# Vasilispapg/CVML-GoalNet

Hardware: AMD Instinct MI355X
Metric: training clips/sec at batch 64, 16-frame 224² clips; logit MAE vs CPU ref (higher is better)
Workload: dtype f32; 1 GPU; AVM train step (forward + broadcast-MSE + backward + fused Adam), 64 clips x 16 frames = 1024 frames of 3x224x224 + 30x30 MFCC per GPU; dropout live (device masks), BatchNorm train mode; frames_per_gpu=1024, h=224, w=224, parallelism=dp1, ddp_semantics=local BN + local MSE per rank, gradient mean (standard DDP), params=1286754369

## Files before the change

__graft_entry__.py:

```python
from __future__ import annotations

import glob
import os
import subprocess
import sys

ROOT = os.path.dirname(os.path.abspath(__file__))
PKG = os.path.join(ROOT, "cvml_goalnet_amd")
CSRC = os.path.join(PKG, "csrc")
LIB = os.path.join(PKG, "libgoalnet_hip.so")
HIPCC = os.environ.get("HIPCC", "/opt/rocm/bin/hipcc")
FLAGS = ["--offload-arch=gfx950", "-O3", "-std=c++17", "-fPIC", "-Wall", "-Wno-unused-function"]


def _stale(target, sources):
    if not os.path.exists(target):
        return True
    t = os.path.getmtime(target)
    return any(os.path.getmtime(s) > t for s in sources)


def build(force: bool = False) -> None:
    srcs = sorted(glob.glob(os.path.join(CSRC, "*.hip")))
    hdrs = sorted(glob.glob(os.path.join(CSRC, "*.h"))) + [os.path.join(ROOT, "include", h) for h in ("goalnet_hip.h", "goalnet_loss.h", "goalnet_epoch.h", "goalnet_optim.h", "goalnet_ema.h")]
    objdir = os.path.join(CSRC, "build")
    os.makedirs(objdir, exist_ok=True)
    objs = []
    procs = []
    for s in srcs:
        o = os.path.join(objdir, os.path.basename(s)[:-4] + ".o")
        objs.append(o)
        if force or _stale(o, [s] + hdrs):
            procs.append((s, subprocess.Popen([HIPCC, *FLAGS, "-c", s, "-o", o])))
    for s, p in procs:
        if p.wait() != 0:
            raise RuntimeError(f"hipcc failed on {s}")
    if force or procs or _stale(LIB, objs):
        subprocess.check_call([HIPCC, "--offload-arch=gfx950", "-shared", "-fPIC", "-o", LIB, *objs])
    if ROOT not in sys.path:
# ... 54 lines not shown
```

cvml_goalnet_amd/_lib.py:

```python
from __future__ import annotations

import ctypes
import os
from ctypes import c_char_p, c_double, c_float, c_int, c_int32, c_int64, c_size_t, c_uint32, c_uint64, c_void_p

_HERE = os.path.dirname(os.path.abspath(__file__))
LIB_PATH = os.environ.get("GOALNET_LIB_PATH") or os.path.join(_HERE, "libgoalnet_hip.so")
ABI_VERSION = 7
STAT_PARTS = 1024
ADAM_RANGES_MAX = 32

P = c_void_p


class RowCopy(ctypes.Structure):
    _fields_ = [("src", c_void_p), ("dst", c_void_p), ("row_bytes", c_int64), ("nrows", c_int), ("gather", c_int), ("cursor", c_void_p),
                ("cursor_bias", c_int64)]


class RowCopyIndexed(ctypes.Structure):
    _fields_ = [("src", c_void_p), ("dst", c_void_p), ("row_bytes", c_int64), ("nrows", c_int), ("gather", c_int), ("cursor", c_void_p),
                ("cursor_bias", c_int64), ("indexed", c_int), ("table_rows", c_int64)]


# ... 173 lines not shown

OPTIM_PROTOTYPES = {
    "goalnet_grad_sumsq_ws_bytes": (c_size_t, [ctypes.POINTER(OptimRange), c_int]),
    "goalnet_grad_sumsq": (c_int, [P, ctypes.POINTER(OptimRange), c_int, P, P, c_size_t, P]),
    "goalnet_optim_step_dev_ranges": (c_int, [P, P, P, P, ctypes.POINTER(OptimRange), c_int, ctypes.POINTER(OptimOpts), P, c_float, P,
                                              P, c_int64, c_int64, c_int, P, P]),
    "goalnet_optim_lr": (c_int, [ctypes.POINTER(OptimOpts), P, P, P]),
}
SCHEDULES = {"constant": 0, "cosine": 1, "step": 2}

EMA_PROTOTYPES = {
    "goalnet_ema_update_dev_ranges": (c_int, [P, P, ctypes.POINTER(AdamRange), c_int, ctypes.POINTER(EmaOpts), P, c_int64, P, P]),
    "goalnet_swap_ranges": (c_int, [P, P, ctypes.POINTER(AdamRange), c_int, P]),
}

_lib = None


class GoalnetError(RuntimeError):
    pass


def load():
    global _lib
    if _lib is not None:
        return _lib
    if not os.path.exists(LIB_PATH):
        raise GoalnetError(
            f"{LIB_PATH} not found: build it with `python -c 'import __graft_entry__ as g; g.build()'`. "
            "There is no CPU / eager fallback for the AVM hot path.")
    lib = ctypes.CDLL(LIB_PATH)
    for name, (res, args) in (*PROTOTYPES.items(), *LOSS_PROTOTYPES.items(), *EPOCH_PROTOTYPES.items(), *OPTIM_PROTOTYPES.items(),
                              *EMA_PROTOTYPES.items()):
        fn = getattr(lib, name)
        fn.restype = res
        fn.argtypes = args
    v = lib.goalnet_abi_version()
    if v != ABI_VERSION:
        raise GoalnetError(f"libgoalnet_hip.so ABI {v} != expected {ABI_VERSION}")
    _lib = lib
    return lib


def check(rc: int, what: str = ""):
    if rc != 0:
        msg = load().goalnet_last_error()
        raise GoalnetError(f"{what}: rc={rc}: {msg.decode() if msg else ''}")
```

cvml_goalnet_amd/avm.py:

```python
from __future__ import annotations

import contextlib
import math
import os
from typing import List, Optional

import torch
import torch.nn as nn
from torch.nn.parameter import UninitializedParameter

from . import ops
from ._lib import GoalnetError
from .synth import BASE_SEED, DROP_P, TID_DROP

F32 = torch.float32
BN_EPS = 1e-5
BN_MOMENTUM = 0.1
_ALIGN = 64


class _LazyFlags:

    def requires_grad_(self, requires_grad: bool = True):
        for p in self.parameters():
# ... 57 lines not shown
            torch.cuda.current_stream().wait_event(ev)

    def join(self):
        if self.enabled and self.forked:
            torch.cuda.current_stream().wait_stream(self.side)
            self.forked = False
        self.keep.clear()


class _Bwd:

    def __init__(self, model, train, fork):
        self.model, self.train, self.fork = model, train, fork
        self.scratch = {}
        self.dbias = {}
        self.T = train.__contains__

    def any_T(self, *layers):
        return any(f"{layer}.{leaf}" in self.train for layer in layers for leaf in ("weight", "bias"))

    def G(self, name):
        m = self.model
        if name in self.train:
            return m._gflat(name)
        s = m.spec(name)
        if s.kind in ("ohwi", "lin5") and name != "visbl.conv1.weight":
            raise GoalnetError(f"a backward that does not train {name} asked for its gradient")
        t = self.scratch.get(name)
        if t is None:
            t = self.scratch[name] = torch.empty(s.numel, dtype=F32, device=m._device)
# ... 32 lines not shown
    if env is None or env in ("", "1"):
        return frozenset("a")
    if env == "0":
        return frozenset()
    return frozenset(ch for ch in env.lower() if ch in "a")


def epi_fuse_dw_adam(n, *, plain, synced, precision, train_w5, shadowed, inspected, forced, pieces):
    if forced is False or "a" not in pieces:
        return False
    if inspected and forced is not True:
        return False
    if not (plain and not synced and precision == "fp32" and train_w5 and not shadowed):
        return False
    if n <= EPI_FUSE_SKINNY_ROWS:
        return False
    return forced is True or n >= EPI_FUSE_MIN_ROWS


def optim_step_path(optim, *, sharded):
    if optim is None or optim.trivial:
        return False
    if sharded:
        raise GoalnetError("optimizer options (weight decay, clipping, schedules) are not built for ddp.GradSync(shard_linear5=True): "
                           "a rank holds only its slice of linear5.weight's gradient; use a plain GradSync")
    return True


def ema_step_path(ema, *, sharded):
    if ema is None:
# ... 85 lines not shown
        self._materialized = False
        self.grad_sync = None
        self.stat_sync = None
        self.grad_bf16 = os.environ.get("GOALNET_DZ16", "1") != "0"
        self.act_bf16 = os.environ.get("GOALNET_P16", "1") != "0"
        env = os.environ.get
        self.x6_off = env("GOALNET_X6_OFF") == "1"
        self.x6_linear5 = env("GOALNET_X6_LINEAR5", "1") != "0"
        self.x3_wgrad2 = env("GOALNET_X3_WGRAD2", "1") != "0"
        self.x3_dgrad2 = env("GOALNET_X3_DGRAD2", "1") != "0"
        self.mlp_fused = env("GOALNET_MLP_FUSED", "1") != "0"
        self.small_bn = env("GOALNET_SMALL_BN", "1") != "0"
        self.force_bf5 = env("GOALNET_FORCE_BF5") == "1"
        self.overlap_pair = env("GOALNET_OVERLAP_PAIR", "1") != "0"
        self.epi_fuse = None
        self.epi_fused_dw = 0
        self.keep_ctx = False
        self.last_ctx = None
        self.last_used_w5b = False
        self._side_stream = None
        self.overlap_rows = int(os.environ.get("GOALNET_OVERLAP_ROWS", "64"))
        _ol = os.environ.get("GOALNET_OVERLAP_LARGE")
        self.overlap_large = _ol == "1"
        self.overlap_auto = _ol is None
        self.time_labels = None
        self.kernel_events = None

    @property
    def precision(self) -> str:
        return self._precision
# ... 543 lines not shown

    def _block_bwd(self, bwd, dbn, ctx, i, n, hc, wc, c):
        dev, G, bias = self._device, bwd.G, bwd.T(f"visbl.conv{i}.bias")
        p, idx, st = ctx[f"p{i}"], ctx[f"idx{i}"], ctx[f"st{i}"]
        npix = n * (hc - 2) * (wc - 2)
        small = self._small_bn(dbn, p, n, hc, wc, c) and not (self._half and i > 1)
        frozen = ctx["eval"]
        if small:
            coef3 = torch.empty(3 * c, dtype=F32, device=dev)
            (ops.bn_bwd_reduce_small_eval if frozen else ops.bn_bwd_reduce_small)(
                dbn, p, st[0], st[1], self._pflat(f"visbl.bnorm{i}.weight"), G(f"visbl.bnorm{i}.weight"), G(f"visbl.bnorm{i}.bias"),
                coef3, n, hc, wc, c)
            dy = torch.empty(n, hc, wc, c, dtype=F32, device=dev)
            dparts = torch.empty(ops.stat_parts(8 * n) * c, dtype=torch.float64, device=dev)
            ops.bnpool_bwd(dbn, p, idx, coef3, dy, dparts, n, hc, wc, c)
            if i > 1 and bias:
                bwd.dbias[i] = (dparts, c)
            return dy
        coef3 = torch.empty(3 * c, dtype=F32, device=dev)
        partials = torch.empty(ops.stat_parts(npix // 64) * 2 * c, dtype=torch.float64, device=dev)
        ops.bn_bwd_reduce(dbn, p, st[0], st[1], partials, npix, c)
        if frozen:
            ops.bn_bwd_finalize_eval(partials, self._pflat(f"visbl.bnorm{i}.weight"), st[1], c,
                                     G(f"visbl.bnorm{i}.weight"), G(f"visbl.bnorm{i}.bias"), coef3)
        else:
            ops.bn_bwd_finalize(partials, self._pflat(f"visbl.bnorm{i}.weight"), st[0], st[1], npix, c,
                                G(f"visbl.bnorm{i}.weight"), G(f"visbl.bnorm{i}.bias"), coef3)
        if self.stat_sync is not None and not frozen:
            scratch = torch.empty(2 * c, dtype=F32, device=dev)
            ops.bn_bwd_finalize(self._global_sums(partials, 2 * c), self._pflat(f"visbl.bnorm{i}.weight"), st[0], st[1],
                                npix * self.stat_sync.world, c, scratch[:c], scratch[c:], coef3)
        dparts = torch.empty(ops.stat_parts(8 * n) * c, dtype=torch.float64, device=dev)
        if self._half and i > 1 and self._bwd16_ok(wc):
            dy = self._padbuf(f"dy{i}", n, hc, wc, c)
            ops.bnpool_bwd_bf16p(dbn, p, idx, coef3, None, dy, dparts, n, hc, wc, c)
        elif self._half and i > 1:
            dy32 = torch.empty(n, hc, wc, c, dtype=F32, device=dev)
            ops.bnpool_bwd(dbn, p, idx, coef3, dy32, dparts, n, hc, wc, c)
            dy = ops.to_bf16_padded(dy32, None, None, self._padbuf(f"dy{i}", n, hc, wc, c), n, hc, wc, c)
        else:
            dy = torch.empty(n, hc, wc, c, dtype=F32, device=dev)
            ops.bnpool_bwd(dbn, p, idx, coef3, dy, dparts, n, hc, wc, c)
        if not bias:
            return dy
        if i == 1:
            ops.partials_sum(dparts, ops.stat_parts(8 * n), c, c, G(f"visbl.conv{i}.bias"))
        else:
# ... 9 lines not shown
        if after_block:
            after_block()
        split = not self._half and xs in ctx
        if not bwd.T(wname):
            wg = None
            if split and split_dgrad and dgrad:
                dys, ady = self._split_act(f"dy{i}s", dy, None, None, n, hc, wc, cout)
        elif self._half:
            wg, keep = (ops.conv3x3_wgrad_bf16, ctx[f"xh{i - 1}"], dy, G(wname), n, hc, wc, cin, cout), (dy,)
        elif split:
            dys, ady = self._split_act(f"dy{i}s", dy, None, None, n, hc, wc, cout)
            osc_w = self._osc(ady, ctx[xs + "_amax"])
            wg, keep = (ops.conv3x3_wgrad_split, self._parts, ctx[xs], dys, G(wname), n, hc, wc, cin, cout, osc_w), (dys, osc_w)
        else:
            st_in = ctx[f"st{i - 1}"]
            wg, keep = (ops.conv3x3_wgrad, ctx[f"p{i - 1}"], st_in[2], st_in[3], dy, G(wname), n, hc, wc, cin, cout), (dy,)

        def wgrad():
            if wg is not None:
                fork.run(lambda: self._timed("conv_wgrad", flops, *wg), *keep)
        if not pair:
            wgrad()
        if not dgrad:
            if pair:
                wgrad()
            return None
        if flipped:
            fork.wait(wait_ev)
        else:
            ops.conv3x3_weight_flip(P(wname), wt, cout, cin)
        o16 = out16 and ops.conv3x3_fwd_bf16p_o16_ok(n, hc, wc, cout, cin)
# ... 24 lines not shown
            train = frozenset(s.name for s in self._specs) - frozen
        if self._half and ctx["padgen"] != (self._padgen["x1"], self._padgen["x2"]):
            raise RuntimeError("precision='bf16': a second training-mode forward overwrote the saved bf16 operands before "
                               "backward ran; call backward after each forward (as the reference's loop does)")
        for i in (3, 2):
            xs = f"x{i - 1}s"
            if not self._half and xs in ctx and f"visbl.conv{i}.weight" in train and ctx[xs + "_gen"] != self._padgen[xs]:
                raise RuntimeError(f"precision='{self.precision}': a second training-mode forward overwrote the saved split operands "
                                   "before backward ran; call backward after each forward (as the reference's loop does)")
        if params:
            self._ensure_garena()
            self._bwd_frozen = frozen
        dev = self._device
        n, h, w = ctx["n"], ctx["h"], ctx["w"]
        bwd = _Bwd(self, train, _Fork(self, self._fork_ok(n) and dout.is_cuda))
        fork, T, G, any_T = bwd.fork, bwd.T, bwd.G, bwd.any_T
        (h1, w1), (hp1, wp1), (hp2, wp2), (hp3, wp3) = self._sizes(h, w)
        P = self._pflat
        need_b1 = need_vis or any_T("visbl.bnorm1", "visbl.conv1")
        need_b2 = need_b1 or any_T("visbl.bnorm2", "visbl.conv2")
        need_b3 = need_b2 or any_T("visbl.bnorm3", "visbl.conv3")
        train_w5 = T("visbl.linear5.weight")
        need_audbl = self.audio_included and (need_aud or any_T("audbl.linear3", "audbl.conv2", "audbl.conv1"))
        need_cat = need_audbl or need_b3 or train_w5 or T("visbl.linear5.bias")
        d_audio = torch.empty(n, 30, ctx["bins"], dtype=F32, device=dev) if need_aud else None
        d_visual = None
        hs, ms = ctx["hs"], ctx["ms"]
        pair = fork.enabled and self._pair(n)
        deferred_l5 = []

# ... 636 lines not shown
```

cvml_goalnet_amd/csrc/gemm_f32.hip:

```cpp
#include <stdlib.h>

#include "adam.h"
#include "gemm_common.h"
#include "skinny.h"

using namespace goalnet;

namespace {

constexpr int BM = 128, BN = 128, BK = 32;
constexpr int LDR = 128;
constexpr int OP_FLOATS = BM * BK;

__device__ __forceinline__ int kc_off(int row, int chunk) { return row * BK + ((chunk ^ ((row >> 1) & 7)) << 2); }

__device__ __forceinline__ float4 f4zero() { return make_float4(0.f, 0.f, 0.f, 0.f); }
__device__ __forceinline__ float4 f4fma(float4 v, float4 s, float4 t) {
    return make_float4(fmaf(v.x, s.x, t.x), fmaf(v.y, s.y, t.y), fmaf(v.z, s.z, t.z), fmaf(v.w, s.w, t.w));
}

typedef unsigned int u32x4 __attribute__((ext_vector_type(4)));
constexpr unsigned OOB = 0xFFFFFF00u;

__device__ __forceinline__ float4 f4sel(bool v, float4 a) { return v ? a : f4zero(); }
// ... 378 lines not shown
        int n = 0;
        for (; n + 3 < N; n += 4) {
            a0 += q[(int64_t)n * 8 * Cout]; a1 += q[(int64_t)(n + 1) * 8 * Cout];
            a2 += q[(int64_t)(n + 2) * 8 * Cout]; a3 += q[(int64_t)(n + 3) * 8 * Cout];
        }
        for (; n < N; ++n) a0 += q[(int64_t)n * 8 * Cout];
    }
    s[cl][j] = (a0 + a1) + (a2 + a3);
    __syncthreads();
    for (int t = threadIdx.x; t < 32 * 9; t += 256) {
        const int cc = t / 9, tap = t - 9 * cc;
        if (blockIdx.x * 32 + cc < Cout) u[(int64_t)(blockIdx.x * 32 + cc) * 9 + tap] = border_u_of(s[cc], tap);
    }
}

template <bool KC>
__device__ __forceinline__ void store_tile(float* l, const float4 (&r)[4], int tid) {
    if (KC) {
        const int c4 = (tid & 7) * 4, row = tid >> 3;
#pragma unroll
        for (int i = 0; i < 4; ++i) *reinterpret_cast<float4*>(&l[kc_off(row + 32 * i, c4 >> 2)]) = r[i];
    } else {
        const int r4 = (tid & 31) * 4, k = tid >> 5;
#pragma unroll
        for (int i = 0; i < 4; ++i) *reinterpret_cast<float4*>(&l[(k + 8 * i) * LDR + r4]) = r[i];
    }
}

template <bool KC>
__device__ __forceinline__ void read_group(const float* l, int strip, int s, int r, int h, float (&f)[2][4]) {
// ... 707 lines not shown
            const int64_t blocks = tiles * c, rounds = (blocks + 511) / 512;
            const double eff = (double)blocks / (double)(rounds * 512);
            if (eff > best_eff + 1e-9) { best_eff = eff; best = c; }
        }
        s = best;
    }
    const int kps = (int)((ktiles + s - 1) / s);
    return (ktiles + kps - 1) / kps;
}

static size_t wgrad_codes_bytes(int64_t M) { return (size_t)((M + 31) / 32 * 32 + 255) / 256 * 256; }
static size_t wgrad_border_bytes(int N, int Cout) {
    return ((size_t)N * 8 * Cout * sizeof(double) + 255) / 256 * 256 + ((size_t)Cout * 9 * sizeof(float) + 255) / 256 * 256;
}

size_t goalnet_conv3x3_wgrad_ws_bytes(int N, int H, int W, int Cin, int Cout) {
    const int64_t M = (int64_t)N * H * W;
    return wgrad_codes_bytes(M) + wgrad_border_bytes(N, Cout) + (size_t)wgrad_splits(M, Cin, Cout) * (size_t)Cout * 9 * Cin * sizeof(float);
}

int goalnet_conv3x3_wgrad_codes(uint32_t* codes, int N, int H, int W, void* stream) {
    GN_REQUIRE(codes && N > 0 && H > 0 && W > 0, GOALNET_E_NULL, "conv3x3_wgrad_codes: bad arguments");
    const int64_t M = (int64_t)N * H * W;
    GN_REQUIRE(M < (1ll << 31) - 256, GOALNET_E_SHAPE, "conv3x3_wgrad_codes: N*H*W too large");
    const int Mpad = (int)((M + 31) / 32 * 32);
    int blocks = (Mpad / 4 + 255) / 256;
    if (blocks > 4096) blocks = 4096;
    hipLaunchKernelGGL(border_codes_kernel, dim3(blocks), dim3(256), 0, (hipStream_t)stream, codes, (int)M, Mpad, H, W);
    GN_LAUNCH_CHECK("conv3x3_wgrad_codes");
    return 0;
// ... 9 lines not shown
    GN_REQUIRE(N > 0 && H > 0 && W > 0, GOALNET_E_SHAPE, "conv3x3_wgrad: non-positive dim");
    GN_REQUIRE(Cin % 4 == 0 && Cout % 4 == 0 && Cin > 0 && Cout > 0, GOALNET_E_SHAPE, "conv3x3_wgrad: channels must be multiples of 4");
    GN_REQUIRE(aligned16(x) && aligned16(dy) && aligned16(dw) && aligned16(ws) && aligned16(scale) && aligned16(shift),
               GOALNET_E_ALIGN, "conv3x3_wgrad: pointers must be 16-byte aligned");
    const int64_t M = (int64_t)N * H * W;
    GN_REQUIRE(M < (1ll << 31) - 256, GOALNET_E_SHAPE, "conv3x3_wgrad: N*H*W too large");
    GN_REQUIRE(ws_bytes >= goalnet_conv3x3_wgrad_ws_bytes(N, H, W, Cin, Cout), GOALNET_E_WORKSPACE, "conv3x3_wgrad: workspace too small");
    hipStream_t st = (hipStream_t)stream;
    const int nsplit = wgrad_splits(M, Cin, Cout);
    const int ktiles = (int)((M + BK - 1) / BK);
    const int64_t slab = (int64_t)Cout * 9 * Cin;
    uint32_t* codes = (uint32_t*)ws;
    double* bparts = (double*)((char*)ws + wgrad_codes_bytes(M));
    float* bu = (float*)((char*)bparts + ((size_t)N * 8 * Cout * sizeof(double) + 255) / 256 * 256);
    float* slabs = (float*)((char*)ws + wgrad_codes_bytes(M) + wgrad_border_bytes(N, Cout));
    const char* force = getenv("GOALNET_WGRAD_PATH");
    const bool dsel = force && force[0] == 's' ? true : force && force[0] == 'c' ? false : (int64_t)N * (H > W ? H : W) <= 4096;
    if (codes_in) {
        codes = const_cast<uint32_t*>(codes_in);
    } else {
        const int Mpad = (int)((M + 31) / 32 * 32);
        int blocks = (Mpad / 4 + 255) / 256;
        if (blocks > 4096) blocks = 4096;
        hipLaunchKernelGGL(border_codes_kernel, dim3(blocks), dim3(256), 0, st, codes, (int)M, Mpad, H, W);
        GN_LAUNCH_CHECK("conv3x3_wgrad.codes");
    }
    if (scale && !dsel) {
        hipLaunchKernelGGL(wgrad_border_sums_kernel, dim3(N), dim3(256), 0, st, dy, bparts, H, W, Cout);
        GN_LAUNCH_CHECK("conv3x3_wgrad.border_sums");
        hipLaunchKernelGGL(wgrad_border_u_kernel, dim3((Cout + 31) / 32), dim3(256), 0, st, bparts, N, Cout, bu);
        GN_LAUNCH_CHECK("conv3x3_wgrad.border_u");
    }
// ... 8 lines not shown
    int rc;
    if (scale && dsel) {
        ConvWgradBLoader<true, true>::P bp{x, H, W, Cin, (int)M, scale, shift, codes};
        rc = launch_gemm<MCLoader<false>, ConvWgradBLoader<true, true>>("conv3x3_wgrad", ap, bp, ep, Cout, 9 * Cin, ktiles, nsplit, 1, st);
    } else if (scale) {
        ConvWgradBLoader<true>::P bp{x, H, W, Cin, (int)M, scale, shift, codes};
        rc = launch_gemm<MCLoader<false>, ConvWgradBLoader<true>>("conv3x3_wgrad", ap, bp, ep, Cout, 9 * Cin, ktiles, nsplit, 1, st);
    } else {
        ConvWgradBLoader<false>::P bp{x, H, W, Cin, (int)M, nullptr, nullptr, codes};
        rc = launch_gemm<MCLoader<false>, ConvWgradBLoader<false>>("conv3x3_wgrad", ap, bp, ep, Cout, 9 * Cin, ktiles, nsplit, 1, st);
    }
    if (rc || fused) return rc;
    EpiP er{EPI_RAW, dw, (int64_t)9 * Cin, Cout, 9 * Cin, nullptr, 0, nullptr, 0, nullptr, 0, 0};
    if (scale && !dsel) { er.corr_u = bu; er.corr_sh = shift; er.corr_C = Cin; }
    return launch_splitk_reduce("conv3x3_wgrad.reduce", slabs, nsplit, slab, er, st);
}

static int linear_splits(int M, int64_t K, int J) {
    const int64_t tiles = (int64_t)((M + BM - 1) / BM) * ((J + BN - 1) / BN);
    return pick_splits(tiles, (int)(K / BK));
}

size_t goalnet_linear_fwd_ws_bytes(int M, int64_t K, int J) {
    if (M <= 0 || K <= 0 || J <= 0) return 0;
    if (M <= SKINNY_MAX_M) return skinny_fwd_ws_bytes(M, K, J);
    const int s = linear_splits(M, K, J);
    return s > 1 ? (size_t)s * (size_t)M * (size_t)J * sizeof(float) : 0;
}

int goalnet_linear_fwd(const float* x, int64_t ldx, const float* scale, const float* shift, int bnC,
// ... 109 lines not shown
```

cvml_goalnet_amd/csrc/pool_bn.hip:

```cpp
#include <hip/hip_bf16.h>
#include <stdlib.h>

#include "common.h"

using namespace goalnet;

namespace {

constexpr int PARTS = GOALNET_STAT_PARTS;

struct d4 { double x, y, z, w; };

template <int NV>
__device__ __forceinline__ void block_reduce_store(double (&v)[NV][4], int G, int tid, double* smem,
                                                   double* out_row, int64_t out_stride, int C) {
#pragma unroll
    for (int a = 0; a < NV; ++a)
#pragma unroll
        for (int c = 0; c < 4; ++c) smem[tid * (NV * 4) + a * 4 + c] = v[a][c];
    __syncthreads();
    if (tid < G) {
        const int reps = 256 / G;
#pragma unroll
        for (int a = 0; a < NV; ++a)
// ... 142 lines not shown
__device__ __forceinline__ float h16_lo(unsigned u) { return (float)__builtin_bit_cast(_Float16, (unsigned short)(u & 0xffffu)); }
__device__ __forceinline__ float h16_hi(unsigned u) { return (float)__builtin_bit_cast(_Float16, (unsigned short)(u >> 16)); }
__device__ __forceinline__ float4 f4_of_h16(const uint2& u) { return make_float4(h16_lo(u.x), h16_hi(u.x), h16_lo(u.y), h16_hi(u.y)); }
__device__ __forceinline__ float4 load_dz4(const _Float16* q) { return f4_of_h16(*reinterpret_cast<const uint2*>(q)); }

__device__ __forceinline__ float4 load_dz4_raw(const float* q) { return *reinterpret_cast<const float4*>(q); }
__device__ __forceinline__ uint2 load_dz4_raw(const __hip_bfloat16* q) { return *reinterpret_cast<const uint2*>(q); }
__device__ __forceinline__ h16raw load_dz4_raw(const _Float16* q) { return h16raw{*reinterpret_cast<const uint2*>(q)}; }
__device__ __forceinline__ float4 dz4_of(const float4& v) { return v; }
__device__ __forceinline__ float4 dz4_of(const uint2& u) {
    return make_float4(__uint_as_float(u.x << 16), __uint_as_float(u.x & 0xffff0000u), __uint_as_float(u.y << 16), __uint_as_float(u.y & 0xffff0000u));
}
__device__ __forceinline__ float4 dz4_of(const h16raw& r) { return f4_of_h16(r.u); }

template <typename DZ, typename PT>
__global__ __launch_bounds__(256) void bn_bwd_reduce_kernel(const DZ* __restrict__ dz, const PT* __restrict__ p,
                                                           const float* __restrict__ mean, const float* __restrict__ invstd,
                                                           double* __restrict__ partials, int64_t npix, int C) {
    __shared__ double smem[256 * 8];
    const int tid = threadIdx.x;
    const int G = C >> 2;
    const int g = tid % G, pl = tid / G;
    const int ppi = 256 / G;
    const float4 mu = *reinterpret_cast<const float4*>(mean + g * 4);
    const float4 is = *reinterpret_cast<const float4*>(invstd + g * 4);
    double acc[2][4] = {{0, 0, 0, 0}, {0, 0, 0, 0}};
    for (int64_t pix = (int64_t)blockIdx.x * ppi + pl; pix < npix; pix += (int64_t)gridDim.x * ppi) {
        const float4 d = load_dz4(dz + pix * C + g * 4);
        const float4 x = load_dz4(p + pix * C + g * 4);
        acc[0][0] += (double)d.x; acc[1][0] += (double)d.x * (double)((x.x - mu.x) * is.x);
        acc[0][1] += (double)d.y; acc[1][1] += (double)d.y * (double)((x.y - mu.y) * is.y);
        acc[0][2] += (double)d.z; acc[1][2] += (double)d.z * (double)((x.z - mu.z) * is.z);
        acc[0][3] += (double)d.w; acc[1][3] += (double)d.w * (double)((x.w - mu.w) * is.w);
    }
    block_reduce_store<2>(acc, G, tid, smem, partials + (int64_t)blockIdx.x * 2 * C, C, C);
}

__global__ __launch_bounds__(256) void bn_bwd_finalize_kernel(const double* __restrict__ partials, const float* __restrict__ gamma,
                                                             const float* __restrict__ mean, const float* __restrict__ invstd,
                                                             double count, int nparts, int C, float* __restrict__ dgamma,
                                                             float* __restrict__ dbeta, float* __restrict__ coef3) {
    __shared__ double sm[256];
    const int c = blockIdx.x * 16 + (threadIdx.x & 15);
    const double s = column_sum16(partials + c, nparts, 2 * C, c < C, sm);
    const double q = column_sum16(partials + C + c, nparts, 2 * C, c < C, sm);
    if (c >= C || threadIdx.x >= 16) return;
    dbeta[c] = (float)s;
    dgamma[c] = (float)q;
    const double a = (double)gamma[c] * (double)invstd[c];
    const double m1 = s / count, m2 = q / count;
// ... 877 lines not shown
    GN_LAUNCH_CHECK("bn_bwd_finalize_eval");
    return 0;
}

int goalnet_bn_bwd_reduce(const float* dz, const float* p, const float* mean, const float* invstd,
                          double* partials, int nparts, int64_t npix, int C, void* stream) {
    GN_REQUIRE(dz && p && mean && invstd && partials, GOALNET_E_NULL, "bn_bwd_reduce: null pointer");
    GN_REQUIRE(npix > 0 && chan_ok(C), GOALNET_E_SHAPE, "bn_bwd_reduce: bad dims");
    GN_PARTS_OK("bn_bwd_reduce");
    GN_REQUIRE(aligned16(dz) && aligned16(p) && aligned16(mean) && aligned16(invstd), GOALNET_E_ALIGN, "bn_bwd_reduce: alignment");
    hipLaunchKernelGGL((bn_bwd_reduce_kernel<float, float>), dim3(nparts), dim3(256), 0, (hipStream_t)stream, dz, p, mean, invstd, partials, npix, C);
    GN_LAUNCH_CHECK("bn_bwd_reduce");
    return 0;
}

int goalnet_bn_bwd_reduce_t(const void* dz, int dz_bf16, const void* p, int p_bf16, const float* mean, const float* invstd,
                            double* partials, int nparts, int64_t npix, int C, int f16, void* stream) {
    GN_REQUIRE(dz && p && mean && invstd && partials, GOALNET_E_NULL, "bn_bwd_reduce_t: null pointer");
    GN_REQUIRE(npix > 0 && chan_ok(C), GOALNET_E_SHAPE, "bn_bwd_reduce_t: bad dims");
    GN_PARTS_OK("bn_bwd_reduce_t");
    GN_REQUIRE(aligned16(dz) && aligned16(p) && aligned16(mean) && aligned16(invstd), GOALNET_E_ALIGN, "bn_bwd_reduce_t: alignment");
    const dim3 grid(nparts), block(256);
    hipStream_t st = (hipStream_t)stream;
    typedef __hip_bfloat16 bf;
    typedef _Float16 hf;
    if (f16 && dz_bf16 && p_bf16) hipLaunchKernelGGL((bn_bwd_reduce_kernel<hf, hf>), grid, block, 0, st, (const hf*)dz, (const hf*)p, mean, invstd, partials, npix, C);
    else if (f16 && dz_bf16)      hipLaunchKernelGGL((bn_bwd_reduce_kernel<hf, float>), grid, block, 0, st, (const hf*)dz, (const float*)p, mean, invstd, partials, npix, C);
    else if (f16 && p_bf16)       hipLaunchKernelGGL((bn_bwd_reduce_kernel<float, hf>), grid, block, 0, st, (const float*)dz, (const hf*)p, mean, invstd, partials, npix, C);
    else if (dz_bf16 && p_bf16) hipLaunchKernelGGL((bn_bwd_reduce_kernel<bf, bf>), grid, block, 0, st, (const bf*)dz, (const bf*)p, mean, invstd, partials, npix, C);
    else if (dz_bf16)      hipLaunchKernelGGL((bn_bwd_reduce_kernel<bf, float>), grid, block, 0, st, (const bf*)dz, (const float*)p, mean, invstd, partials, npix, C);
// ... 178 lines not shown
```

cvml_goalnet_amd/ops.py:

```python
from __future__ import annotations

import ctypes
import os

import torch

from . import _lib
from ._lib import STAT_PARTS, check

F32 = torch.float32


def _s():
    return torch.cuda.current_stream().cuda_stream


def _p(t):
    return 0 if t is None else t.data_ptr()


def _chk(*ts):
    for t in ts:
        if t is None:
            continue
# ... 117 lines not shown
    check(lib().goalnet_bn_finalize(partials.data_ptr(), _rows(partials, 2 * C), gamma.data_ptr(), beta.data_ptr(), _p(rmean), _p(rvar), momentum, eps,
                                    count, C, mean.data_ptr(), invstd.data_ptr(), scale.data_ptr(), shift.data_ptr(), _s()),
          "bn_finalize")


def bn_bwd_reduce(dz, p, mean, invstd, partials, npix, C):
    _chk(dz, p, mean, invstd, partials)
    _req(dz.numel() == p.numel() == npix * C, "bn_bwd_reduce: argument check failed: dz.numel() == p.numel() == npix * C")
    if dz.dtype in H16 or p.dtype in H16:
        check(lib().goalnet_bn_bwd_reduce_t(dz.data_ptr(), int(dz.dtype in H16), p.data_ptr(), int(p.dtype in H16),
                                            mean.data_ptr(), invstd.data_ptr(), partials.data_ptr(), _rows(partials, 2 * C), npix, C,
                                            _f16(dz, p), _s()), "bn_bwd_reduce_t")
        return
    check(lib().goalnet_bn_bwd_reduce(dz.data_ptr(), p.data_ptr(), mean.data_ptr(), invstd.data_ptr(), partials.data_ptr(),
                                      _rows(partials, 2 * C), npix, C, _s()), "bn_bwd_reduce")


def bn_bwd_finalize(partials, gamma, mean, invstd, count, C, dgamma, dbeta, coef3):
    _chk(partials, gamma, mean, invstd, dgamma, dbeta, coef3)
    _req(coef3.numel() == 3 * C and dgamma.numel() == C and dbeta.numel() == C, "bn_bwd_finalize: argument check failed: coef3.numel() == 3 * C and dgamma.numel() == C and dbeta.numel() == C")
    check(lib().goalnet_bn_bwd_finalize(partials.data_ptr(), _rows(partials, 2 * C), gamma.data_ptr(), mean.data_ptr(), invstd.data_ptr(), count, C,
                                        dgamma.data_ptr(), dbeta.data_ptr(), coef3.data_ptr(), _s()), "bn_bwd_finalize")


def bnpool_bwd(dz, p, idx, coef3, dy, dbias_partials, N, Hc, Wc, C):
    _chk(dz, p, idx, coef3, dy, dbias_partials)
    npool = N * (Hc - 2) * (Wc - 2) * C
    _req(dz.numel() == p.numel() == idx.numel() == npool and dy.numel() == N * Hc * Wc * C, "bnpool_bwd: argument check failed: dz.numel() == p.numel() == idx.numel() == npool and dy.numel() == N * Hc * Wc * C")
    if dz.dtype in H16 or p.dtype in H16:
        check(lib().goalnet_bnpool_bwd_bf16p_t(dz.data_ptr(), int(dz.dtype in H16), p.data_ptr(), int(p.dtype in H16),
# ... 128 lines not shown


def conv3x3_fwd(x, scale, shift, w, bias, relu, y, N, H, W, Cin, Cout):
    _chk(x, scale, shift, w, bias, y)
    _req(x.numel() == N * H * W * Cin and y.numel() == N * H * W * Cout and w.numel() == Cout * 9 * Cin, "conv3x3_fwd: argument check failed: x.numel() == N * H * W * Cin and y.numel() == N * H * W * Cout and w.numel() == Cout * 9 * Cin")
    _req(scale is None or (scale.numel() == Cin and shift.numel() == Cin), "conv3x3_fwd: argument check failed: scale is None or (scale.numel() == Cin and shift.numel() == Cin)")
    _req(bias is None or bias.numel() == Cout, "conv3x3_fwd: argument check failed: bias is None or bias.numel() == Cout")
    nbytes = lib().goalnet_conv3x3_fwd_ws_bytes(N, H, W, Cin, Cout)
    ws = torch.empty(nbytes // 4, dtype=F32, device=x.device) if nbytes else None
    ctr = _tile_counters(("conv3x3_fwd", N, H, W, Cin, Cout, scale is None), x.device) if (nbytes and FUSED_SPLITK) else None
    check(lib().goalnet_conv3x3_fwd(x.data_ptr(), _p(scale), _p(shift), w.data_ptr(), _p(bias), int(relu), y.data_ptr(),
                                    N, H, W, Cin, Cout, _p(ws), nbytes, _p(ctr), N_TILE_CTR if ctr is not None else 0, _s()), "conv3x3_fwd")
    return y


def conv3x3_wgrad(x, scale, shift, dy, dw, N, H, W, Cin, Cout):
    _chk(x, scale, shift, dy, dw)
    _req(x.numel() == N * H * W * Cin and dy.numel() == N * H * W * Cout and dw.numel() == Cout * 9 * Cin, "conv3x3_wgrad: argument check failed: x.numel() == N * H * W * Cin and dy.numel() == N * H * W * Cout and dw.numel() == Cout * 9 * Cin")
    nbytes = lib().goalnet_conv3x3_wgrad_ws_bytes(N, H, W, Cin, Cout)
    ws = torch.empty(nbytes // 4, dtype=F32, device=x.device)
    ck = (N, H, W, x.device.index)
    codes = _WGRAD_CODES.get(ck)
    if codes is None:
        codes = torch.empty(lib().goalnet_conv3x3_wgrad_codes_bytes(N, H, W) // 4, dtype=torch.int32, device=x.device)
        check(lib().goalnet_conv3x3_wgrad_codes(codes.data_ptr(), N, H, W, _s()), "conv3x3_wgrad_codes")
        if len(_WGRAD_CODES) < 64 and N * H * W <= (1 << 22):
            _WGRAD_CODES[ck] = codes
    ctr = _tile_counters(("conv3x3_wgrad", N, H, W, Cin, Cout), x.device) if FUSED_SPLITK else None
    check(lib().goalnet_conv3x3_wgrad(x.data_ptr(), _p(scale), _p(shift), dy.data_ptr(), dw.data_ptr(), ws.data_ptr(), nbytes,
                                      codes.data_ptr(), _p(ctr), N_TILE_CTR if ctr is not None else 0, N, H, W, Cin, Cout, _s()), "conv3x3_wgrad")
    return dw


BF16 = torch.bfloat16
F16 = torch.float16
H16 = (BF16, F16)
ADAM_RANGES_MAX = _lib.ADAM_RANGES_MAX


def _f16(*ts):
    kinds = {t.dtype for t in ts if t is not None and t.dtype in H16}
    _req(len(kinds) <= 1, "_f16: 16-bit operands of one call must share a format")
    return int(F16 in kinds)


# ... 805 lines not shown
```

Baseline: 161.7 clips/s.

## Derive BN backward sums from next conv's weights and wgrad instead of rereading activations

For visual blocks 1 and 2, the BatchNorm backward reduction (sum of dz and sum of dz*xhat) is rebuilt algebraically. It uses the following conv's weights, its weight gradient, the dy tap totals and the border sums already held in the wgrad workspace. This skips a full pass over the large activation and gradient tensors. A device-side flag checks that scale is finite and nonzero and that |beta| <= |gamma|; when the check fails, a gated fallback kernel runs the original reduction, so the cheap path runs only when the identity is numerically safe. The cost is extra small kernels, extra workspace, and some risk of numerical drift in fp64 sums.

```diff
diff --git a/__graft_entry__.py b/__graft_entry__.py
--- a/__graft_entry__.py
+++ b/__graft_entry__.py
@@ -22,7 +22,7 @@
 
 def build(force: bool = False) -> None:
     srcs = sorted(glob.glob(os.path.join(CSRC, "*.hip")))
-    hdrs = sorted(glob.glob(os.path.join(CSRC, "*.h"))) + [os.path.join(ROOT, "include", h) for h in ("goalnet_hip.h", "goalnet_loss.h", "goalnet_epoch.h", "goalnet_optim.h", "goalnet_ema.h")]
+    hdrs = sorted(glob.glob(os.path.join(CSRC, "*.h"))) + [os.path.join(ROOT, "include", h) for h in ("goalnet_hip.h", "goalnet_loss.h", "goalnet_epoch.h", "goalnet_optim.h", "goalnet_ema.h", "goalnet_bnsums.h")]
     objdir = os.path.join(CSRC, "build")
     os.makedirs(objdir, exist_ok=True)
     objs = []
diff --git a/cvml_goalnet_amd/_lib.py b/cvml_goalnet_amd/_lib.py
--- a/cvml_goalnet_amd/_lib.py
+++ b/cvml_goalnet_amd/_lib.py
@@ -211,6 +211,14 @@
     "goalnet_swap_ranges": (c_int, [P, P, ctypes.POINTER(AdamRange), c_int, P]),
 }
 
+BNSUMS_PROTOTYPES = {
+    "goalnet_conv3x3_wgrad_border_off": (c_int64, [c_int, c_int, c_int]),
+    "goalnet_bn_sums_max_ratio": (c_float, []),
+    "goalnet_bn_sums_conv_ws_bytes": (c_size_t, [c_int, c_int, c_int]),
+    "goalnet_bn_sums_conv": (c_int, [P, P, P, c_int, P, P, P, P, P, P, P, P, P, c_int, P, P, c_size_t, c_int, c_int, c_int, c_int, c_int, P]),
+    "goalnet_bn_bwd_reduce_gated": (c_int, [P, P, P, P, P, c_int, c_int64, c_int, P, P]),
+}
+
 _lib = None
 
 
@@ -228,7 +236,7 @@
             "There is no CPU / eager fallback for the AVM hot path.")
     lib = ctypes.CDLL(LIB_PATH)
     for name, (res, args) in (*PROTOTYPES.items(), *LOSS_PROTOTYPES.items(), *EPOCH_PROTOTYPES.items(), *OPTIM_PROTOTYPES.items(),
-                              *EMA_PROTOTYPES.items()):
+                              *EMA_PROTOTYPES.items(), *BNSUMS_PROTOTYPES.items()):
         fn = getattr(lib, name)
         fn.restype = res
         fn.argtypes = args
diff --git a/cvml_goalnet_amd/avm.py b/cvml_goalnet_amd/avm.py
--- a/cvml_goalnet_amd/avm.py
+++ b/cvml_goalnet_amd/avm.py
@@ -95,6 +95,9 @@
         self.model, self.train, self.fork = model, train, fork
         self.scratch = {}
         self.dbias = {}
+        self.synced = False
+        self.sums = {}
+        self.tparts = {}
         self.T = train.__contains__
 
     def any_T(self, *layers):
@@ -157,6 +160,17 @@
     if not (plain and not synced and precision == "fp32" and train_w5 and not shadowed):
         return False
     if n <= EPI_FUSE_SKINNY_ROWS:
+        return False
+    return forced is True or n >= EPI_FUSE_MIN_ROWS
+
+
+BN_SUMS_BLOCKS = (1, 2)
+
+
+def bn_sums_route(n, block, *, precision, synced, stat_synced, eval_bn, train_consumer, small, forked, forced, enabled):
+    if forced is False or not enabled or block not in BN_SUMS_BLOCKS:
+        return False
+    if precision != "fp32" or synced or stat_synced or eval_bn or not train_consumer or small or forked:
         return False
     return forced is True or n >= EPI_FUSE_MIN_ROWS
 
@@ -272,6 +286,9 @@
         self.force_bf5 = env("GOALNET_FORCE_BF5") == "1"
         self.overlap_pair = env("GOALNET_OVERLAP_PAIR", "1") != "0"
         self.epi_fuse = None
+        self.bn_sums = None
+        self.bn_sums_enabled = env("GOALNET_BN_SUMS", "1") != "0"
+        self.bn_sums_blocks = 0
         self.epi_fused_dw = 0
         self.keep_ctx = False
         self.last_ctx = None
@@ -845,12 +862,25 @@
             dy = torch.empty(n, hc, wc, c, dtype=F32, device=dev)
             dparts = torch.empty(ops.stat_parts(8 * n) * c, dtype=torch.float64, device=dev)
             ops.bnpool_bwd(dbn, p, idx, coef3, dy, dparts, n, hc, wc, c)
+            bwd.tparts[i] = dparts
             if i > 1 and bias:
                 bwd.dbias[i] = (dparts, c)
             return dy
         coef3 = torch.empty(3 * c, dtype=F32, device=dev)
         partials = torch.empty(ops.stat_parts(npix // 64) * 2 * c, dtype=torch.float64, device=dev)
-        ops.bn_bwd_reduce(dbn, p, st[0], st[1], partials, npix, c)
+        src = bwd.sums.pop(i, None)
+        if src is not None and bn_sums_route(n, i, precision=self.precision, synced=bwd.synced, stat_synced=self.stat_sync is not None,
+                                             eval_bn=frozen, train_consumer=True, small=False, forked=bwd.fork.enabled,
+                                             forced=self.bn_sums, enabled=self.bn_sums_enabled):
+            flag = torch.empty(1, dtype=torch.int32, device=dev)
+            ops.bn_sums_conv(src["w"], src["dw"], src["tparts"], self._pflat(f"visbl.bnorm{i}.weight"), self._pflat(f"visbl.bnorm{i}.bias"),
+                             st, partials, flag, n, hc - 2, wc - 2, c, src["cout"],
+                             border=src["border"][0] if src["border"] else None, dy=src["dy"])
+            ops.bn_bwd_reduce_gated(dbn, p, st[0], st[1], partials, npix, c, flag)
+            self.bn_sums_blocks += 1
+        else:
+            ops.bn_bwd_reduce(dbn, p, st[0], st[1], partials, npix, c)
+        del src
         if frozen:
             ops.bn_bwd_finalize_eval(partials, self._pflat(f"visbl.bnorm{i}.weight"), st[1], c,
                                      G(f"visbl.bnorm{i}.weight"), G(f"visbl.bnorm{i}.bias"), coef3)
@@ -862,6 +892,7 @@
             ops.bn_bwd_finalize(self._global_sums(partials, 2 * c), self._pflat(f"visbl.bnorm{i}.weight"), st[0], st[1],
                                 npix * self.stat_sync.world, c, scratch[:c], scratch[c:], coef3)
         dparts = torch.empty(ops.stat_parts(8 * n) * c, dtype=torch.float64, device=dev)
+        bwd.tparts[i] = dparts
         if self._half and i > 1 and self._bwd16_ok(wc):
             dy = self._padbuf(f"dy{i}", n, hc, wc, c)
             ops.bnpool_bwd_bf16p(dbn, p, idx, coef3, None, dy, dparts, n, hc, wc, c)
@@ -901,7 +932,10 @@
             wg, keep = (ops.conv3x3_wgrad_split, self._parts, ctx[xs], dys, G(wname), n, hc, wc, cin, cout, osc_w), (dys, osc_w)
         else:
             st_in = ctx[f"st{i - 1}"]
-            wg, keep = (ops.conv3x3_wgrad, ctx[f"p{i - 1}"], st_in[2], st_in[3], dy, G(wname), n, hc, wc, cin, cout), (dy,)
+            border = []
+            wg, keep = (ops.conv3x3_wgrad, ctx[f"p{i - 1}"], st_in[2], st_in[3], dy, G(wname), n, hc, wc, cin, cout, border), (dy,)
+            if dgrad and self.bn_sums is not False and self.bn_sums_enabled and not fork.enabled:
+                bwd.sums[i - 1] = dict(w=P(wname), dw=G(wname), tparts=bwd.tparts[i], border=border, dy=dy, cout=cout)
 
         def wgrad():
             if wg is not None:
@@ -956,6 +990,7 @@
         dev = self._device
         n, h, w = ctx["n"], ctx["h"], ctx["w"]
         bwd = _Bwd(self, train, _Fork(self, self._fork_ok(n) and dout.is_cuda))
+        bwd.synced = self.grad_sync is not None or on_bucket is not None
         fork, T, G, any_T = bwd.fork, bwd.T, bwd.G, bwd.any_T
         (h1, w1), (hp1, wp1), (hp2, wp2), (hp3, wp3) = self._sizes(h, w)
         P = self._pflat
diff --git a/cvml_goalnet_amd/csrc/gemm_f32.hip b/cvml_goalnet_amd/csrc/gemm_f32.hip
--- a/cvml_goalnet_amd/csrc/gemm_f32.hip
+++ b/cvml_goalnet_amd/csrc/gemm_f32.hip
@@ -1,5 +1,6 @@
 #include <stdlib.h>
 
+#include "../../include/goalnet_bnsums.h"
 #include "adam.h"
 #include "gemm_common.h"
 #include "skinny.h"
@@ -416,6 +417,109 @@
     }
 }
 
+constexpr float BN_SUMS_MAX_RATIO = 1.0f;
+constexpr int BN_SUMS_ROWS = 64;
+
+__global__ __launch_bounds__(1024) void bn_sums_tu_kernel(const double* __restrict__ t_parts, int t_nparts, const double* __restrict__ bparts,
+                                                         int N, int Cout, double* __restrict__ tu) {
+    __shared__ double s[4][32][8], st[32][32];
+    const int cl = threadIdx.x & 31, j = (threadIdx.x >> 5) & 7, q = threadIdx.x >> 8;
+    const int c = blockIdx.x * 32 + cl;
+    double a0 = 0, a1 = 0, a2 = 0, a3 = 0, t = 0;
+    if (c < Cout) {
+        const double* b = bparts + (int64_t)j * Cout + c;
+        const int per = (N + 3) / 4, n0 = q * per, n1 = n0 + per < N ? n0 + per : N;
+        int n = n0;
+        for (; n + 3 < n1; n += 4) {
+            a0 += b[(int64_t)n * 8 * Cout]; a1 += b[(int64_t)(n + 1) * 8 * Cout];
+            a2 += b[(int64_t)(n + 2) * 8 * Cout]; a3 += b[(int64_t)(n + 3) * 8 * Cout];
+        }
+        for (; n < n1; ++n) a0 += b[(int64_t)n * 8 * Cout];
+        for (int row = 8 * q + j; row < t_nparts; row += 32) t += t_parts[(int64_t)row * Cout + c];
+    }
+    s[q][cl][j] = (a0 + a1) + (a2 + a3);
+    st[cl][8 * q + j] = t;
+    __syncthreads();
+    for (int i = threadIdx.x; i < 32 * 9; i += 1024) {
+        const int cc = i / 9, tap = i - 9 * cc;
+        if (blockIdx.x * 32 + cc >= Cout) continue;
+        double v[8];
+#pragma unroll
+        for (int k = 0; k < 8; ++k) v[k] = (s[0][cc][k] + s[1][cc][k]) + (s[2][cc][k] + s[3][cc][k]);
+        const int kh = tap / 3, kw = tap - 3 * kh;
+        double u = (kh == 0 ? v[0] : 0.0) + (kh == 2 ? v[1] : 0.0) + (kw == 0 ? v[2] : 0.0) + (kw == 2 ? v[3] : 0.0);
+        if (kh == 0 && kw == 0) u -= v[4];
+        if (kh == 0 && kw == 2) u -= v[5];
+        if (kh == 2 && kw == 0) u -= v[6];
+        if (kh == 2 && kw == 2) u -= v[7];
+        double T = 0.0;
+        for (int k = 0; k < 32; ++k) T += st[cc][k];
+        tu[(int64_t)(blockIdx.x * 32 + cc) * 9 + tap] = T - u;
+    }
+}
+
+__global__ __launch_bounds__(256) void bn_sums_conv_kernel(const float* __restrict__ w, const float* __restrict__ dw,
+                                                          const double* __restrict__ tu, int R, int Cin, double* __restrict__ sparts) {
+    __shared__ double smem[256 * 8];
+    const int tid = threadIdx.x;
+    const int G = Cin >> 2, g = tid % G, pl = tid / G, lanes = 256 / G;
+    const int row0 = blockIdx.x * BN_SUMS_ROWS;
+    const int row1 = row0 + BN_SUMS_ROWS < R ? row0 + BN_SUMS_ROWS : R;
+    double acc[2][4] = {{0, 0, 0, 0}, {0, 0, 0, 0}};
+    for (int row = row0 + pl; row < row1; row += lanes) {
+        const float4 a = *reinterpret_cast<const float4*>(w + (int64_t)row * Cin + g * 4);
+        const float4 d = *reinterpret_cast<const float4*>(dw + (int64_t)row * Cin + g * 4);
+        const double t = tu[row];
+        acc[0][0] = fma((double)a.x, t, acc[0][0]); acc[1][0] += (double)a.x * (double)d.x;
+        acc[0][1] = fma((double)a.y, t, acc[0][1]); acc[1][1] += (double)a.y * (double)d.y;
+        acc[0][2] = fma((double)a.z, t, acc[0][2]); acc[1][2] += (double)a.z * (double)d.z;
+        acc[0][3] = fma((double)a.w, t, acc[0][3]); acc[1][3] += (double)a.w * (double)d.w;
+    }
+#pragma unroll
+    for (int v = 0; v < 2; ++v)
+#pragma unroll
+        for (int c = 0; c < 4; ++c) smem[tid * 8 + v * 4 + c] = acc[v][c];
+    __syncthreads();
+    if (tid < G) {
+        double* out = sparts + (int64_t)blockIdx.x * 2 * Cin;
+#pragma unroll
+        for (int v = 0; v < 2; ++v)
+#pragma unroll
+            for (int c = 0; c < 4; ++c) {
+                double sum = 0.0;
+                for (int rp = 0; rp < lanes; ++rp) sum += smem[(rp * G + tid) * 8 + v * 4 + c];
+                out[(int64_t)v * Cin + tid * 4 + c] = sum;
+            }
+    }
+}
+
+struct BnSumsCoef {
+    const float* gamma; const float* beta; const float* mean; const float* invstd; const float* scale; const float* shift;
+};
+
+__global__ __launch_bounds__(256) void bn_sums_finish_kernel(const double* __restrict__ sparts, int nsp, BnSumsCoef k, int C,
+                                                            double* __restrict__ partials, int nparts, int* __restrict__ flag) {
+    int bad = 0;
+    for (int c = threadIdx.x; c < C; c += 256) {
+        const float sc = k.scale[c];
+        bad |= !(sc != 0.f && fabsf(sc) <= 3.0e38f) || !(fabsf(k.beta[c]) <= BN_SUMS_MAX_RATIO * fabsf(k.gamma[c]));
+    }
+    bad = __syncthreads_or(bad);
+    if (blockIdx.x == 0) {
+        for (int c = threadIdx.x; c < C; c += 256) {
+            double s1 = 0.0, s2 = 0.0;
+            for (int b = 0; b < nsp; ++b) { s1 += sparts[(int64_t)b * 2 * C + c]; s2 += sparts[(int64_t)b * 2 * C + C + c]; }
+            const double sc = (double)k.scale[c], sh = (double)k.shift[c], mu = (double)k.mean[c], is = (double)k.invstd[c];
+            partials[c] = s1;
+            partials[C + c] = is * ((s2 - sh * s1) / sc - mu * s1);
+        }
+        if (threadIdx.x == 0) *flag = bad ? 1 : 0;
+    }
+    const int64_t nz = (int64_t)(nparts - 1) * 2 * C;
+    double* z = partials + 2 * C;
+    for (int64_t i = (int64_t)blockIdx.x * 256 + threadIdx.x; i < nz; i += (int64_t)gridDim.x * 256) z[i] = 0.0;
+}
+
 template <bool KC>
 __device__ __forceinline__ void store_tile(float* l, const float4 (&r)[4], int tid) {
     if (KC) {
@@ -1153,6 +1257,11 @@
     return ((size_t)N * 8 * Cout * sizeof(double) + 255) / 256 * 256 + ((size_t)Cout * 9 * sizeof(float) + 255) / 256 * 256;
 }
 
+static bool wgrad_dsel(int N, int H, int W) {
+    const char* force = getenv("GOALNET_WGRAD_PATH");
+    return force && force[0] == 's' ? true : force && force[0] == 'c' ? false : (int64_t)N * (H > W ? H : W) <= 4096;
+}
+
 size_t goalnet_conv3x3_wgrad_ws_bytes(int N, int H, int W, int Cin, int Cout) {
     const int64_t M = (int64_t)N * H * W;
     return wgrad_codes_bytes(M) + wgrad_border_bytes(N, Cout) + (size_t)wgrad_splits(M, Cin, Cout) * (size_t)Cout * 9 * Cin * sizeof(float);
@@ -1192,8 +1301,7 @@
     double* bparts = (double*)((char*)ws + wgrad_codes_bytes(M));
     float* bu = (float*)((char*)bparts + ((size_t)N * 8 * Cout * sizeof(double) + 255) / 256 * 256);
     float* slabs = (float*)((char*)ws + wgrad_codes_bytes(M) + wgrad_border_bytes(N, Cout));
-    const char* force = getenv("GOALNET_WGRAD_PATH");
-    const bool dsel = force && force[0] == 's' ? true : force && force[0] == 'c' ? false : (int64_t)N * (H > W ? H : W) <= 4096;
+    const bool dsel = wgrad_dsel(N, H, W);
     if (codes_in) {
         codes = const_cast<uint32_t*>(codes_in);
     } else {
@@ -1232,6 +1340,53 @@
     EpiP er{EPI_RAW, dw, (int64_t)9 * Cin, Cout, 9 * Cin, nullptr, 0, nullptr, 0, nullptr, 0, 0};
     if (scale && !dsel) { er.corr_u = bu; er.corr_sh = shift; er.corr_C = Cin; }
     return launch_splitk_reduce("conv3x3_wgrad.reduce", slabs, nsplit, slab, er, st);
+}
+
+int64_t goalnet_conv3x3_wgrad_border_off(int N, int H, int W) {
+    if (N <= 0 || H <= 0 || W <= 0 || wgrad_dsel(N, H, W)) return -1;
+    return (int64_t)wgrad_codes_bytes((int64_t)N * H * W);
+}
+
+size_t goalnet_bn_sums_conv_ws_bytes(int N, int Cin, int Cout) {
+    if (N <= 0 || Cin <= 0 || Cout <= 0) return 0;
+    const size_t nsp = ((size_t)Cout * 9 + BN_SUMS_ROWS - 1) / BN_SUMS_ROWS;
+    return ((size_t)N * 8 * Cout + (size_t)Cout * 9 + nsp * 2 * Cin) * sizeof(double);
+}
+
+float goalnet_bn_sums_max_ratio(void) { return BN_SUMS_MAX_RATIO; }
+
+int goalnet_bn_sums_conv(const float* w, const float* dw, const double* t_parts, int t_nparts, const double* border_parts,
+                         const float* dy, const float* gamma, const float* beta, const float* mean, const float* invstd,
+                         const float* scale, const float* shift, double* partials, int nparts, int* flag,
+                         void* ws, size_t ws_bytes, int N, int H, int W, int Cin, int Cout, void* stream) {
+    GN_REQUIRE(w && dw && t_parts && (border_parts || dy) && gamma && beta && mean && invstd && scale && shift && partials && flag && ws,
+               GOALNET_E_NULL, "bn_sums_conv: null pointer");
+    GN_REQUIRE(N > 0 && H > 0 && W > 0 && Cout > 0 && Cout % 4 == 0, GOALNET_E_SHAPE, "bn_sums_conv: bad dims");
+    GN_REQUIRE(Cin >= 4 && Cin <= 1024 && (Cin & (Cin - 1)) == 0, GOALNET_E_SHAPE, "bn_sums_conv: Cin=%d must be a power of two in [4, 1024]", Cin);
+    GN_REQUIRE(t_nparts >= 1 && nparts >= 1 && nparts <= GOALNET_STAT_PARTS, GOALNET_E_SHAPE, "bn_sums_conv: bad partial-row counts");
+    GN_REQUIRE(aligned16(w) && aligned16(dw) && aligned16(ws) && aligned16(partials), GOALNET_E_ALIGN, "bn_sums_conv: alignment");
+    GN_REQUIRE(ws_bytes >= goalnet_bn_sums_conv_ws_bytes(N, Cin, Cout), GOALNET_E_WORKSPACE, "bn_sums_conv: workspace too small");
+    hipStream_t st = (hipStream_t)stream;
+    const int R = Cout * 9, nsp = (R + BN_SUMS_ROWS - 1) / BN_SUMS_ROWS;
+    double* bp = (double*)ws;
+    double* tu = bp + (size_t)N * 8 * Cout;
+    double* sparts = tu + (size_t)Cout * 9;
+    if (!border_parts) {
+        hipLaunchKernelGGL(wgrad_border_sums_kernel, dim3(N), dim3(256), 0, st, dy, bp, H, W, Cout);
+        GN_LAUNCH_CHECK("bn_sums_conv.border_sums");
+        border_parts = bp;
+    }
+    hipLaunchKernelGGL(bn_sums_tu_kernel, dim3((Cout + 31) / 32), dim3(1024), 0, st, t_parts, t_nparts, border_parts, N, Cout, tu);
+    GN_LAUNCH_CHECK("bn_sums_conv.tu");
+    hipLaunchKernelGGL(bn_sums_conv_kernel, dim3(nsp), dim3(256), 0, st, w, dw, tu, R, Cin, sparts);
+    GN_LAUNCH_CHECK("bn_sums_conv.sums");
+    const int64_t nz = (int64_t)(nparts - 1) * 2 * Cin;
+    int fin = (int)((nz + 256 * 8 - 1) / (256 * 8));
+    fin = fin < 1 ? 1 : fin > 256 ? 256 : fin;
+    const BnSumsCoef k{gamma, beta, mean, invstd, scale, shift};
+    hipLaunchKernelGGL(bn_sums_finish_kernel, dim3(fin), dim3(256), 0, st, sparts, nsp, k, Cin, partials, nparts, flag);
+    GN_LAUNCH_CHECK("bn_sums_conv.finish");
+    return 0;
 }
 
 static int linear_splits(int M, int64_t K, int J) {
diff --git a/cvml_goalnet_amd/csrc/pool_bn.hip b/cvml_goalnet_amd/csrc/pool_bn.hip
--- a/cvml_goalnet_amd/csrc/pool_bn.hip
+++ b/cvml_goalnet_amd/csrc/pool_bn.hip
@@ -1,6 +1,7 @@
 #include <hip/hip_bf16.h>
 #include <stdlib.h>
 
+#include "../../include/goalnet_bnsums.h"
 #include "common.h"
 
 using namespace goalnet;
@@ -180,10 +181,9 @@
 __device__ __forceinline__ float4 dz4_of(const h16raw& r) { return f4_of_h16(r.u); }
 
 template <typename DZ, typename PT>
-__global__ __launch_bounds__(256) void bn_bwd_reduce_kernel(const DZ* __restrict__ dz, const PT* __restrict__ p,
-                                                           const float* __restrict__ mean, const float* __restrict__ invstd,
-                                                           double* __restrict__ partials, int64_t npix, int C) {
-    __shared__ double smem[256 * 8];
+__device__ __forceinline__ void bn_bwd_reduce_body(const DZ* __restrict__ dz, const PT* __restrict__ p,
+                                                   const float* __restrict__ mean, const float* __restrict__ invstd,
+                                                   double* __restrict__ partials, int64_t npix, int C, double* smem) {
     const int tid = threadIdx.x;
     const int G = C >> 2;
     const int g = tid % G, pl = tid / G;
@@ -200,6 +200,23 @@
         acc[0][3] += (double)d.w; acc[1][3] += (double)d.w * (double)((x.w - mu.w) * is.w);
     }
     block_reduce_store<2>(acc, G, tid, smem, partials + (int64_t)blockIdx.x * 2 * C, C, C);
+}
+
+template <typename DZ, typename PT>
+__global__ __launch_bounds__(256) void bn_bwd_reduce_kernel(const DZ* __restrict__ dz, const PT* __restrict__ p,
+                                                           const float* __restrict__ mean, const float* __restrict__ invstd,
+                                                           double* __restrict__ partials, int64_t npix, int C) {
+    __shared__ double smem[256 * 8];
+    bn_bwd_reduce_body(dz, p, mean, invstd, partials, npix, C, smem);
+}
+
+__global__ __launch_bounds__(256) void bn_bwd_reduce_gated_kernel(const float* __restrict__ dz, const float* __restrict__ p,
+                                                                 const float* __restrict__ mean, const float* __restrict__ invstd,
+                                                                 double* __restrict__ partials, int64_t npix, int C,
+                                                                 const int* __restrict__ gate) {
+    __shared__ double smem[256 * 8];
+    if (*gate == 0) return;
+    bn_bwd_reduce_body(dz, p, mean, invstd, partials, npix, C, smem);
 }
 
 __global__ __launch_bounds__(256) void bn_bwd_finalize_kernel(const double* __restrict__ partials, const float* __restrict__ gamma,
@@ -1107,6 +1124,17 @@
     return 0;
 }
 
+int goalnet_bn_bwd_reduce_gated(const float* dz, const float* p, const float* mean, const float* invstd,
+                                double* partials, int nparts, int64_t npix, int C, const int* gate, void* stream) {
+    GN_REQUIRE(dz && p && mean && invstd && partials && gate, GOALNET_E_NULL, "bn_bwd_reduce_gated: null pointer");
+    GN_REQUIRE(npix > 0 && chan_ok(C), GOALNET_E_SHAPE, "bn_bwd_reduce_gated: bad dims");
+    GN_PARTS_OK("bn_bwd_reduce_gated");
+    GN_REQUIRE(aligned16(dz) && aligned16(p) && aligned16(mean) && aligned16(invstd), GOALNET_E_ALIGN, "bn_bwd_reduce_gated: alignment");
+    hipLaunchKernelGGL(bn_bwd_reduce_gated_kernel, dim3(nparts), dim3(256), 0, (hipStream_t)stream, dz, p, mean, invstd, partials, npix, C, gate);
+    GN_LAUNCH_CHECK("bn_bwd_reduce_gated");
+    return 0;
+}
+
 int goalnet_bn_bwd_reduce_t(const void* dz, int dz_bf16, const void* p, int p_bf16, const float* mean, const float* invstd,
                             double* partials, int nparts, int64_t npix, int C, int f16, void* stream) {
     GN_REQUIRE(dz && p && mean && invstd && partials, GOALNET_E_NULL, "bn_bwd_reduce_t: null pointer");
diff --git a/cvml_goalnet_amd/ops.py b/cvml_goalnet_amd/ops.py
--- a/cvml_goalnet_amd/ops.py
+++ b/cvml_goalnet_amd/ops.py
@@ -155,6 +155,38 @@
         return
     check(lib().goalnet_bn_bwd_reduce(dz.data_ptr(), p.data_ptr(), mean.data_ptr(), invstd.data_ptr(), partials.data_ptr(),
                                       _rows(partials, 2 * C), npix, C, _s()), "bn_bwd_reduce")
+
+
+def bn_sums_max_ratio():
+    return float(lib().goalnet_bn_sums_max_ratio())
+
+
+def bn_sums_conv(w, dw, t_parts, gamma, beta, st, partials, flag, N, H, W, Cin, Cout, border=None, dy=None):
+    _chk(w, dw, t_parts, gamma, beta, *st, partials, flag, dy)
+    _req(w.numel() == dw.numel() == Cout * 9 * Cin and w.dtype == dw.dtype == F32, "bn_sums_conv: w, dw fp32 of Cout * 9 * Cin elements")
+    _req(gamma.numel() == Cin and beta.numel() == Cin and all(s.numel() == Cin and s.dtype == F32 for s in st) and len(st) == 4,
+         "bn_sums_conv: gamma, beta, mean, invstd, scale, shift (Cin)")
+    _req(flag.dtype == torch.int32 and flag.numel() >= 1, "bn_sums_conv: flag is int32[1]")
+    _req(border is not None or (dy is not None and dy.dtype == F32 and dy.numel() == N * H * W * Cout), "bn_sums_conv: border sums or an fp32 dy")
+    bptr = 0
+    if border is not None:
+        bws, off = border
+        _req(off >= 0 and off % 16 == 0 and bws.numel() * bws.element_size() >= off + N * 8 * Cout * 8, "bn_sums_conv: border sums outside their workspace")
+        bptr = bws.data_ptr() + off
+    nbytes = lib().goalnet_bn_sums_conv_ws_bytes(N, Cin, Cout)
+    ws = torch.empty(nbytes // 8, dtype=torch.float64, device=w.device)
+    check(lib().goalnet_bn_sums_conv(w.data_ptr(), dw.data_ptr(), t_parts.data_ptr(), _rows(t_parts, Cout), bptr, _p(dy), gamma.data_ptr(),
+                                     beta.data_ptr(), st[0].data_ptr(), st[1].data_ptr(), st[2].data_ptr(), st[3].data_ptr(),
+                                     partials.data_ptr(), _rows(partials, 2 * Cin), flag.data_ptr(), ws.data_ptr(), nbytes,
+                                     N, H, W, Cin, Cout, _s()), "bn_sums_conv")
+
+
+def bn_bwd_reduce_gated(dz, p, mean, invstd, partials, npix, C, gate):
+    _chk(dz, p, mean, invstd, partials, gate)
+    _req(dz.dtype == F32 and p.dtype == F32 and dz.numel() == p.numel() == npix * C, "bn_bwd_reduce_gated: fp32 dz, p of npix * C elements")
+    _req(gate.dtype == torch.int32 and gate.numel() >= 1, "bn_bwd_reduce_gated: gate is int32[1]")
+    check(lib().goalnet_bn_bwd_reduce_gated(dz.data_ptr(), p.data_ptr(), mean.data_ptr(), invstd.data_ptr(), partials.data_ptr(),
+                                            _rows(partials, 2 * C), npix, C, gate.data_ptr(), _s()), "bn_bwd_reduce_gated")
 
 
 def bn_bwd_finalize(partials, gamma, mean, invstd, count, C, dgamma, dbeta, coef3):
@@ -313,7 +345,7 @@
     return y
 
 
-def conv3x3_wgrad(x, scale, shift, dy, dw, N, H, W, Cin, Cout):
+def conv3x3_wgrad(x, scale, shift, dy, dw, N, H, W, Cin, Cout, border=None):
     _chk(x, scale, shift, dy, dw)
     _req(x.numel() == N * H * W * Cin and dy.numel() == N * H * W * Cout and dw.numel() == Cout * 9 * Cin, "conv3x3_wgrad: argument check failed: x.numel() == N * H * W * Cin and dy.numel() == N * H * W * Cout and dw.numel() == Cout * 9 * Cin")
     nbytes = lib().goalnet_conv3x3_wgrad_ws_bytes(N, H, W, Cin, Cout)
@@ -328,6 +360,10 @@
     ctr = _tile_counters(("conv3x3_wgrad", N, H, W, Cin, Cout), x.device) if FUSED_SPLITK else None
     check(lib().goalnet_conv3x3_wgrad(x.data_ptr(), _p(scale), _p(shift), dy.data_ptr(), dw.data_ptr(), ws.data_ptr(), nbytes,
                                       codes.data_ptr(), _p(ctr), N_TILE_CTR if ctr is not None else 0, N, H, W, Cin, Cout, _s()), "conv3x3_wgrad")
+    if border is not None and scale is not None:
+        off = lib().goalnet_conv3x3_wgrad_border_off(N, H, W)
+        if off >= 0:
+            border.append((ws, off))
     return dw
 
 
diff --git a/include/goalnet_bnsums.h b/include/goalnet_bnsums.h
--- /dev/null
+++ b/include/goalnet_bnsums.h
@@ -0,0 +1,26 @@
+#ifndef GOALNET_BNSUMS_H
+#define GOALNET_BNSUMS_H
+
+#include "goalnet_hip.h"
+
+#ifdef __cplusplus
+extern "C" {
+#endif
+
+int64_t goalnet_conv3x3_wgrad_border_off(int N, int H, int W);
+
+float goalnet_bn_sums_max_ratio(void);
+
+size_t goalnet_bn_sums_conv_ws_bytes(int N, int Cin, int Cout);
+int goalnet_bn_sums_conv(const float* w, const float* dw, const double* t_parts, int t_nparts, const double* border_parts,
+                         const float* dy, const float* gamma, const float* beta, const float* mean, const float* invstd,
+                         const float* scale, const float* shift, double* partials, int nparts, int* flag,
+                         void* ws, size_t ws_bytes, int N, int H, int W, int Cin, int Cout, void* stream);
+
+int goalnet_bn_bwd_reduce_gated(const float* dz, const float* p, const float* mean, const float* invstd,
+                                double* partials, int nparts, int64_t npix, int C, const int* gate, void* stream);
+
+#ifdef __cplusplus
+}
+#endif
+#endif
```

Result: no change. 162.7 clips/s, median of 6 (+0.6%).
